# zhangxiaochen95/uav_bs_ctrl

Hardware: AMD Instinct MI355X
Metric: env-steps/sec (MADRQN, 8 UBS x 80 GT) (higher is better)
Workload: dtype f32

## Files before the change

include/uavgnn.h:

```cpp
#ifndef UAVGNN_H
#define UAVGNN_H

#include <stddef.h>
#include <stdint.h>

#ifdef __cplusplus
extern "C" {
#endif

#define UAVGNN_VERSION 101

#define UAVGNN_EINVAL (-1000)
#define UAVGNN_EUNSUPPORTED (-1001)
#define UAVGNN_EWORKSPACE (-1002)

typedef void* uavgnn_stream_t;

int uavgnn_version(void);

const char* uavgnn_strerror(int code);

int uavgnn_gatv2_fwd(const float* x_src, int E, int F_src, const float* x_dst, int F_dst, const int32_t* seg_off,
                     const int32_t* dst_order, int N, const float* W_s, const float* b_s, const float* W_d, const float* b_d, const float* attn,
                     const float* W_r, const float* b_r, int nh, int D, float slope, float* out, int ld_out,
// ... 117 lines not shown
int uavgnn_gemm_nt_h2(const float* X, int ldx, int K1, const float* X2, int ldx2, int M, int K, const float* rowmax, const float* rowmax2,
                      const void* planes, int N, const float* bias, float* Y, int ldy, int epilogue, uavgnn_stream_t stream);
int uavgnn_gemm_nt_h2_rm2(const float* X, int ldx, int K1, const float* X2, int ldx2, int M, int K, const float* rowmax, float* rowmax2_out,
                          const void* planes, int N, const float* bias, float* Y, int ldy, int epilogue, uavgnn_stream_t stream);
int uavgnn_gemm_nt_h2_n64(const float* X, int ldx, int M, int K, const float* rowmax, const void* planes, int N, float* Y, int ldy,
                          uavgnn_stream_t stream);
int uavgnn_gru_gates_bwd_fused_sums_rowmax(const float* pre, const float* h, const float* d_hout, const float* dq, int n_out,
                                           const float* W_out, int N, int H, float* d_gi, float* d_gh, float* d_h, float* col_sums,
                                           float* row_absmax, uavgnn_stream_t stream);
int uavgnn_relu_bwd_colsum_rowmax(const float* dy, long long ld, const float* y, long long ldy, float* out, long long ldo, int N, int C,
                                  float* acc, int S, float* row_absmax, uavgnn_stream_t stream);
int uavgnn_relu_bwd_colsum(const float* dy, long long ld, const float* y, long long ldy, float* out, long long ldo, int N, int C,
                           float* acc, int S, uavgnn_stream_t stream);

int uavgnn_flat_obs_supported(int H_out, int F);
int uavgnn_flat_obs_fwd(const float* agent, long long ld_a, int F_a, const float* gt, long long ld_g, int K_g, const float* ubs,
                        long long ld_u, int K_u, int rows, const float* W, const float* b, int H_out, float* y, long long ld_y,
                        uavgnn_stream_t stream);
int uavgnn_flat_obs_wgrad_chunks(long long rows, int H_out, int F);
int uavgnn_flat_obs_wgrad(const float* dy, long long ld_dy, int H_out, const float* agent, long long ld_a, int F_a, const float* gt,
                          long long ld_g, int K_g, const float* ubs, long long ld_u, int K_u, int rows, float* partials, int S,
                          int accumulate, uavgnn_stream_t stream);

int uavgnn_talk_attn_env_supported(int n_max, int M, int K);
int uavgnn_talk_attn_env_fwd(const float* s, int ld_s, const float* q, int ld_q, const float* v, int ld_v, int K, int M,
                             const int32_t* talk_off, const int32_t* talk_src, const int32_t* graph_off, int B,
                             int n_max, float scale, float* c, int ld_c, float* a_save, const float* x_copy, int ld_x,
                             int n_copy, uavgnn_stream_t stream);
int uavgnn_talk_attn_env_bwd(const float* s, int ld_s, const float* q, int ld_q, const float* v, int ld_v, int K, int M,
                             const int32_t* talk_off, const int32_t* talk_src, const int32_t* graph_off, int B,
                             int n_max, float scale, const float* a_save, const float* d_c, int ld_dc, float* d_s,
                             int ld_ds, float* d_q, int ld_dq, float* d_v, int ld_dv, uavgnn_stream_t stream);

int uavgnn_tarmac_msg_supported(int H, int M, int K, int n_ag);
long long uavgnn_tarmac_msg_weight_bytes(int H, int M, int K);
int uavgnn_tarmac_msg_prepare(const float* Wp, int ld, int H, int M, int K, void* tiles, uavgnn_stream_t stream);
int uavgnn_tarmac_msg_fwd(const float* x, int ld_x, const float* h, int ld_h, int N, int H, int n_ag, const void* tiles,
                          const float* bias, int M, int K, const int32_t* talk_off, const int32_t* talk_src, float scale,
                          float* c_out, int ld_c, float* a_save, float* proj_out, int ld_p, float* x_copy, int ld_xc,
                          uavgnn_stream_t stream);
int uavgnn_tarmac_msg_rowmax_supported(int H, int M, int K, int n_ag);
int uavgnn_tarmac_msg_fwd_rowmax(const float* x, int ld_x, const float* h, int ld_h, int N, int H, int n_ag, const void* tiles,
                                 const float* bias, int M, int K, const int32_t* talk_off, const int32_t* talk_src, float scale,
                                 float* c_out, int ld_c, float* a_save, float* proj_out, int ld_p, float* x_copy, int ld_xc,
                                 float* row_absmax, uavgnn_stream_t stream);

size_t uavgnn_degree_order_workspace_bytes(int N);
int uavgnn_degree_order(const int32_t* seg_off, int N, int32_t* order, void* workspace, size_t workspace_bytes,
                        uavgnn_stream_t stream);
size_t uavgnn_csc_transpose_workspace_bytes(int N);
int uavgnn_csc_transpose(const int32_t* talk_off, const int32_t* talk_src, int N, int E, int32_t* t_off,
                         int32_t* t_dst, int32_t* t_pos, void* workspace, size_t workspace_bytes,
                         uavgnn_stream_t stream);
int uavgnn_csc_transpose_env(const int32_t* talk_off, const int32_t* talk_src, const int32_t* graph_off, int B, int N,
                             int32_t* t_off, int32_t* t_dst, int32_t* t_pos, uavgnn_stream_t stream);

int uavgnn_adamw_polyak(float* p, float* g, float* exp_avg, float* exp_avg_sq, float* p_targ, long long n,
                        long long n_clip, const float* hyper, double beta1, double beta2, float eps, float weight_decay,
                        float clip, float polyak, uavgnn_stream_t stream);

int uavgnn_env_state_dim(int n_ubs, int n_gts, int fair_service);
int uavgnn_env_step(const int32_t* int_consts, const double* f64_consts, int B, const long long* actions,
                    const double* avail_moves, double* pos_ubs, const float* pos_gts, int32_t* prior, float* avg_rate,
                    int32_t* t, float* run_f32, double* n_colls, float* d_u2g, float* d_u2u, int32_t* gt_ubs,
                    int32_t* gt_rb, float* rate_per_gt, double* rate_per_ubs, int32_t* mask_collision, double* reward,
                    float* done, float* obs_gt, float* obs_ubs, float* obs_agent, float* state, uavgnn_stream_t stream);
// ... 105 lines not shown
```

uav_bs_ctrl_amd/csrc/f16x2.h:

```cpp
#pragma once
#include <hip/hip_runtime.h>

namespace uavgnn {
namespace h2 {

typedef float f32x2 __attribute__((ext_vector_type(2)));
typedef float f32x16 __attribute__((ext_vector_type(16)));
typedef _Float16 f16x2 __attribute__((ext_vector_type(2)));
typedef _Float16 f16x8 __attribute__((ext_vector_type(8)));
typedef unsigned u32x4 __attribute__((ext_vector_type(4)));
typedef unsigned u32x2 __attribute__((ext_vector_type(2)));

__device__ __forceinline__ int swz32(int row) { return (row >> 2) & 3; }
__device__ __forceinline__ f16x8 as_frag(u32x4 v) { return __builtin_bit_cast(f16x8, v); }
__device__ __forceinline__ f32x16 mfma32(f16x8 a, f16x8 b, f32x16 c) { return __builtin_amdgcn_mfma_f32_32x32x16_f16(a, b, c, 0, 0, 0); }

__device__ __forceinline__ int scale_exp(float amax) {
  const int e = static_cast<int>((__float_as_uint(amax) >> 23) & 0xffu);
  return max(-126, min(126, 14 - (e - 127)));
}
__device__ __forceinline__ float pow2f(int e) { return __uint_as_float(static_cast<unsigned>(e + 127) << 23); }

struct Split2 {
  unsigned hi, lo;
};
__device__ __forceinline__ Split2 split_pair(float x, float y) {
  Split2 s;
  const f16x2 h = __builtin_convertvector(f32x2{x, y}, f16x2);
  s.hi = __builtin_bit_cast(unsigned, h);
  const f32x2 r = f32x2{x, y} - __builtin_convertvector(h, f32x2);
  s.lo = __builtin_bit_cast(unsigned, __builtin_convertvector(r, f16x2));
  return s;
}
__device__ __forceinline__ void stage4(unsigned short* p, int plane_stride, float4 v, float s) {
  const Split2 a = split_pair(v.x * s, v.y * s), b = split_pair(v.z * s, v.w * s);
  *reinterpret_cast<u32x2*>(p) = u32x2{a.hi, b.hi};
  *reinterpret_cast<u32x2*>(p + plane_stride) = u32x2{a.lo, b.lo};
}
__device__ __forceinline__ void stage4(unsigned short* p, int plane_stride, float4 v, float4 s) {
  const Split2 a = split_pair(v.x * s.x, v.y * s.y), b = split_pair(v.z * s.z, v.w * s.w);
  *reinterpret_cast<u32x2*>(p) = u32x2{a.hi, b.hi};
  *reinterpret_cast<u32x2*>(p + plane_stride) = u32x2{a.lo, b.lo};
}

}
}
```

uav_bs_ctrl_amd/csrc/tarmac_msg.hip:

```cpp
#include <math.h>

#include "bf16x3.h"
#include "common.h"

namespace uavgnn {
namespace {

using namespace x3;

constexpr int kMsgWaves = 4;
constexpr int kMsgRows = 16 * kMsgWaves;
constexpr int kMsgThreads = kWave * kMsgWaves;
constexpr int kMaxCols = 128;

__device__ __forceinline__ bf16x8 frag_of(unsigned a, unsigned b, unsigned c, unsigned d) {
  return __builtin_bit_cast(bf16x8, u32x4{a, b, c, d});
}

__device__ __forceinline__ void lds_barrier() {
  __builtin_amdgcn_fence(__ATOMIC_RELEASE, "workgroup", "local");
  __builtin_amdgcn_s_barrier();
  __builtin_amdgcn_fence(__ATOMIC_ACQUIRE, "workgroup", "local");
}

struct Planes8 {
  u32x4 p[3];
};

__device__ __forceinline__ Planes8 split8(const float4 lo, const float4 hi) {
  const Split3 a = split_pair(lo.x, lo.y), b = split_pair(lo.z, lo.w), c = split_pair(hi.x, hi.y), d = split_pair(hi.z, hi.w);
  Planes8 r;
  r.p[0] = u32x4{a.h1, b.h1, c.h1, d.h1};
  r.p[1] = u32x4{a.h2, b.h2, c.h2, d.h2};
  r.p[2] = u32x4{a.h3, b.h3, c.h3, d.h3};
  return r;
}

__global__ __launch_bounds__(256) void tarmac_msg_prepare_kernel(const float* __restrict__ W, int ld, int R, int RP, int KK,
                                                                 u32x4* __restrict__ tiles) {
  const int idx = blockIdx.x * 256 + threadIdx.x;
  const int per_slice = RP * 4, nsl = KK / 32;
  if (idx >= nsl * per_slice) return;
  const int s = idx / per_slice, rem = idx - s * per_slice, r = rem >> 2, c = rem & 3;
  Planes8 pl;
  if (r < R) {
// ... 202 lines not shown
      }
      wave_sync_lds();
      msg_scatter(AD, NA, AV, SRC, DST, OFF, E, lane);
      wave_sync_lds();
      for (int c0 = 0; c0 < M; c0 += kWave) {
        const int ch = c0 + lane, chc = ch < M ? ch : M - 1;
        float v[NA];
#pragma unroll
        for (int t = 0; t < NA; ++t) v[t] = P[t * LDP + chc];
#pragma unroll 4
        for (int r = 0; r < NA; ++r) {
          float a = 0.f;
#pragma unroll
          for (int t = 0; t < NA; t += 4) {
            const float4 q = *reinterpret_cast<const float4*>(AD + r * NA + t);
            a = fmaf(q.x, v[t], a);
            a = fmaf(q.y, v[t + 1], a);
            a = fmaf(q.z, v[t + 2], a);
            a = fmaf(q.w, v[t + 3], a);
          }
          if (ch < M) P[r * LDP + ch] = a;
        }
      }
    }
  }
  wave_sync_lds();
  for (int r = 0; r < 16; ++r) {
    if (row0 + r >= N) break;
    float* d = c_out + static_cast<size_t>(row0 + r) * ld_c;
    for (int ch = lane; ch < M; ch += kWave) d[ch] = P[r * LDP + ch];
  }
}

template <int CT, bool TRAIN, bool RM = false>
__global__ __launch_bounds__(2 * kMsgThreads, 4) void tarmac_msg_fwd_k2_kernel(
    const float* __restrict__ x, int ld_x, const float* __restrict__ h, int ld_h, int N, int H, int n_ag,
    const u32x4* __restrict__ Wt, const float* __restrict__ bias, int M, int K, const int32_t* __restrict__ talk_off,
    const int32_t* __restrict__ talk_src, float scale, float* __restrict__ c_out, int ld_c, float* __restrict__ a_save,
    float* __restrict__ proj_out, int ld_p, float* __restrict__ x_copy, int ld_xc, float* __restrict__ row_absmax = nullptr) {
  constexpr int kThreads = 2 * kMsgThreads;
  __shared__ float sRowMax[kMsgWaves][2][16];
  float amax = 0.f;
  constexpr int RP = 16 * CT;
  constexpr int BCH = 3 * RP * 4;
  constexpr int BPT = (2 * BCH + kThreads - 1) / kThreads;
  constexpr int LDP = RP + 1;
  constexpr int NA = 16, EMAX = NA * NA;
  constexpr int kScratch = (NA + 4) + 5 * EMAX;
  constexpr int kLoopBytes = 2 * 2 * BCH * 16, kTailBytes = kMsgWaves * (16 * LDP + kScratch) * 4;
  __shared__ __attribute__((aligned(16))) unsigned char smem_raw[kLoopBytes > kTailBytes ? kLoopBytes : kTailBytes];
  u32x4(*sB)[2 * BCH] = reinterpret_cast<u32x4(*)[2 * BCH]>(smem_raw);

  const int tid = threadIdx.x, lane = tid & 63;
  const int wave = __builtin_amdgcn_readfirstlane(tid >> 6);
  const int tile = wave & 3, half = wave >> 2;
  const int j = lane & 15, g = lane >> 4;
  const int row0 = blockIdx.x * kMsgRows + tile * 16;
  const int row = row0 + j, rowc = min(row, N - 1);
  const int nsx = H / 32;
  const float* __restrict__ ar = (half ? h + static_cast<size_t>(rowc) * ld_h : x + static_cast<size_t>(rowc) * ld_x) + 4 * g;

  f32x4 acc[CT];
#pragma unroll
  for (int ct = 0; ct < CT; ++ct) acc[ct] = f32x4{0.f, 0.f, 0.f, 0.f};

  u32x4 rb[BPT];
  auto load_b = [&](int t) {
    t = min(t, nsx - 1);
// ... 66 lines not shown
    UAVGNN_MSG_STEP(a1_lo, a1_hi, t + 1)
  }
#undef UAVGNN_MSG_STEP
#undef UAVGNN_MSG_TERM
#undef UAVGNN_MSG_LOAD_A

  float* __restrict__ P = reinterpret_cast<float*>(smem_raw) + tile * (16 * LDP + kScratch);
  const int ncol = M + 2 * K;
  if (RM) load_fsrc();
  if (RM) {
    amax = fmaxf(amax, __shfl_xor(amax, 16));
    amax = fmaxf(amax, __shfl_xor(amax, 32));
    if (g == 0) sRowMax[tile][half][j] = amax;
  }
  if (half == 0) {
#pragma unroll
    for (int ct = 0; ct < CT; ++ct) {
      const int col = ct * 16 + j;
      const float b = col < ncol ? bias[col] : 0.f;
#pragma unroll
      for (int i = 0; i < 4; ++i) P[(4 * g + i) * LDP + col] = acc[ct][i] + b;
    }
  }
  lds_barrier();
  if (half == 1) {
#pragma unroll
    for (int ct = 0; ct < CT; ++ct) {
      const int col = ct * 16 + j;
#pragma unroll
      for (int i = 0; i < 4; ++i) P[(4 * g + i) * LDP + col] += acc[ct][i];
    }
  }
  lds_barrier();
  int* __restrict__ OFF = reinterpret_cast<int*>(P + 16 * LDP);
  float* __restrict__ SC = reinterpret_cast<float*>(OFF + NA + 4);
  float* __restrict__ AD = SC + EMAX;
  int* __restrict__ SRC = reinterpret_cast<int*>(AD + EMAX);
  int* __restrict__ DST = SRC + EMAX;
  float* __restrict__ AV = reinterpret_cast<float*>(DST + EMAX);
  if (half == 1) {
    if (TRAIN && proj_out != nullptr) {
      for (int r = 0; r < 16; ++r) {
        if (row0 + r >= N) break;
        float* d = proj_out + static_cast<size_t>(row0 + r) * ld_p;
        for (int col = lane; col < ncol; col += kWave) d[col] = P[r * LDP + col];
      }
    }
    lds_barrier();
    return;
  }
  bool poison = !ok;
  if (ok) {
    for (int i = lane; i < EMAX; i += kWave) AD[i] = 0.f;
    if (lane <= 16) OFF[lane] = toff - e_lo;
    wave_sync_lds();
    bool bad = false;
#pragma unroll
    for (int i = 0; i < 4; ++i) {
      const int e = lane + kWave * i;
      if (e < E) {
        const int u = fsrc[i] - row0;
        bad |= (u < 0) | (u >= 16);
        SRC[e] = u < 0 ? 0 : (u >= 16 ? 15 : u);
        int d = 0;
#pragma unroll
        for (int jj = 1; jj < 16; ++jj) d += e >= OFF[jj];
        DST[e] = d;
      }
    }
    poison = __any(bad);
    wave_sync_lds();
    if (!poison) {
      for (int e = lane; e < E; e += kWave) {
        const float* __restrict__ sr = P + SRC[e] * LDP + M;
        const float* __restrict__ qr = P + DST[e] * LDP + M + K;
        float a = 0.f;
#pragma unroll 4
        for (int k = 0; k < K; ++k) a = fmaf(sr[k], qr[k], a);
        SC[e] = a * scale;
      }
      wave_sync_lds();
      for (int e = lane; e < E; e += kWave) {
        const int d = DST[e];
        const int j0 = OFF[d], j1 = OFF[d + 1];
        float m = -INFINITY;
#pragma unroll 2
        for (int jj = j0; jj < j1; ++jj) m = fmaxf(m, SC[jj]);
        float den = 0.f;
#pragma unroll 2
        for (int jj = j0; jj < j1; ++jj) den += expf(SC[jj] - m);
        const float a = expf(SC[e] - m) / den;
        if (TRAIN && a_save != nullptr) a_save[e_lo + e] = a;
        AV[e] = a;
      }
      wave_sync_lds();
      msg_scatter(AD, NA, AV, SRC, DST, OFF, E, lane);
      wave_sync_lds();
    }
  }
  lds_barrier();
  if (poison) {
    for (int i = 0; i < 16; ++i)
      for (int ch = lane; ch < M; ch += kWave) P[i * LDP + ch] = NAN;
  } else {
    for (int c0 = 0; c0 < M; c0 += kWave) {
      const int ch = c0 + lane, chc = ch < M ? ch : M - 1;
      float v[NA];
#pragma unroll
      for (int t = 0; t < NA; ++t) v[t] = P[t * LDP + chc];
#pragma unroll 4
      for (int r = 0; r < NA; ++r) {
        float a = 0.f;
#pragma unroll
        for (int t = 0; t < NA; t += 4) {
          const float4 q = *reinterpret_cast<const float4*>(AD + r * NA + t);
          a = fmaf(q.x, v[t], a);
          a = fmaf(q.y, v[t + 1], a);
          a = fmaf(q.z, v[t + 2], a);
          a = fmaf(q.w, v[t + 3], a);
        }
        if (ch < M) P[r * LDP + ch] = a;
      }
    }
  }
  wave_sync_lds();
  for (int r = 0; r < 16; ++r) {
    if (row0 + r >= N) break;
    float* d = c_out + static_cast<size_t>(row0 + r) * ld_c;
    for (int ch = lane; ch < M; ch += kWave) d[ch] = P[r * LDP + ch];
  }
  if (RM) {
    float cm = 0.f;
    for (int ch = g; ch < M; ch += 4) cm = fmaxf(cm, fabsf(P[j * LDP + ch]));
    cm = fmaxf(cm, __shfl_xor(cm, 16));
    cm = fmaxf(cm, __shfl_xor(cm, 32));
    if (g == 0 && row < N) row_absmax[row] = fmaxf(cm, fmaxf(sRowMax[tile][0][j], sRowMax[tile][1][j]));
  }
}

}
}

using namespace uavgnn;

extern "C" int uavgnn_tarmac_msg_supported(int H, int M, int K, int n_ag) {
  if (H < 32 || (H % 32) || M < 1 || K < 1 || K > 64 || M + 2 * K > kMaxCols) return 0;
  if (n_ag < 1 || n_ag > 16 || (16 % n_ag)) return 0;
  return 1;
}

static int msg_rows_padded(int M, int K) {
  const int ct = (M + 2 * K + 15) / 16;
  return 16 * (ct <= 4 ? 4 : ct <= 6 ? 6 : 8);
}

extern "C" long long uavgnn_tarmac_msg_weight_bytes(int H, int M, int K) {
  if (H <= 0 || M <= 0 || K <= 0 || M + 2 * K > kMaxCols) return 0;
  return static_cast<long long>(2 * H / 32) * 3 * msg_rows_padded(M, K) * 64;
}

extern "C" int uavgnn_tarmac_msg_prepare(const float* Wp, int ld, int H, int M, int K, void* tiles, uavgnn_stream_t stream) {
  if (!Wp || !tiles || H <= 0 || M <= 0 || K <= 0 || ld < 2 * H) return UAVGNN_EINVAL;
  if ((H % 32) || (ld & 3) || (reinterpret_cast<uintptr_t>(Wp) & 15) || (reinterpret_cast<uintptr_t>(tiles) & 15) || M + 2 * K > kMaxCols)
    return UAVGNN_EUNSUPPORTED;
  const int R = M + 2 * K, RP = msg_rows_padded(M, K), KK = 2 * H;
  const int total = (KK / 32) * RP * 4;
  hipLaunchKernelGGL(tarmac_msg_prepare_kernel, dim3((total + 255) / 256), dim3(256), 0, static_cast<hipStream_t>(stream), Wp, ld,
                     R, RP, KK, static_cast<u32x4*>(tiles));
  return launch_status();
}

static int msg_launch(const float* x, int ld_x, const float* h, int ld_h, int N, int H, int n_ag, const void* tiles, const float* bias, int M,
                      int K, const int32_t* talk_off, const int32_t* talk_src, float scale, float* c_out, int ld_c, float* a_save,
                      float* proj_out, int ld_p, float* x_copy, int ld_xc, float* row_absmax, uavgnn_stream_t stream) {
  if (N < 0 || !x || !h || !tiles || !bias || !talk_off || !c_out || ld_x < H || ld_h < H || ld_c < M) return UAVGNN_EINVAL;
  if (proj_out && ld_p < M + 2 * K) return UAVGNN_EINVAL;
  if (x_copy && ld_xc < H) return UAVGNN_EINVAL;
  if (!uavgnn_tarmac_msg_supported(H, M, K, n_ag) || (N % n_ag) || (ld_x & 3) || (ld_h & 3) || (x_copy && (ld_xc & 3)) ||
      ((reinterpret_cast<uintptr_t>(x) | reinterpret_cast<uintptr_t>(h) | reinterpret_cast<uintptr_t>(tiles) |
        reinterpret_cast<uintptr_t>(x_copy)) & 15))
    return UAVGNN_EUNSUPPORTED;
  if (N == 0) return 0;
  const int ct = (M + 2 * K + 15) / 16;
  const bool train = a_save != nullptr || proj_out != nullptr || x_copy != nullptr;
  const dim3 grid((N + kMsgRows - 1) / kMsgRows), block(kMsgThreads);
  hipStream_t st = static_cast<hipStream_t>(stream);
  const u32x4* Wt = static_cast<const u32x4*>(tiles);
  if (row_absmax != nullptr && ct > 6) return UAVGNN_EUNSUPPORTED;
  if (ct <= 6) {
    const dim3 block2(2 * kMsgThreads);
#define UAVGNN_MSG_K2(CT_, TR_)                                                                                                        \
  {                                                                                                                                    \
    if (row_absmax != nullptr)                                                                                                         \
      hipLaunchKernelGGL((tarmac_msg_fwd_k2_kernel<CT_, TR_, true>), grid, block2, 0, st, x, ld_x, h, ld_h, N, H, n_ag, Wt, bias, M, K, \
                         talk_off, talk_src, scale, c_out, ld_c, a_save, proj_out, ld_p, x_copy, ld_xc, row_absmax);                   \
    else                                                                                                                               \
      hipLaunchKernelGGL((tarmac_msg_fwd_k2_kernel<CT_, TR_, false>), grid, block2, 0, st, x, ld_x, h, ld_h, N, H, n_ag, Wt, bias, M, K, \
                         talk_off, talk_src, scale, c_out, ld_c, a_save, proj_out, ld_p, x_copy, ld_xc, nullptr);                      \
  }
    if (ct <= 4) {
      if (train) UAVGNN_MSG_K2(4, true)
      else UAVGNN_MSG_K2(4, false)
    } else {
      if (train) UAVGNN_MSG_K2(6, true)
      else UAVGNN_MSG_K2(6, false)
    }
#undef UAVGNN_MSG_K2
    return launch_status();
  }
#define UAVGNN_MSG_K1(TR_)                                                                                                   \
  hipLaunchKernelGGL((tarmac_msg_fwd_kernel<TR_>), grid, block, 0, st, x, ld_x, h, ld_h, N, H, n_ag, Wt, bias, M, K, talk_off, \
                     talk_src, scale, c_out, ld_c, a_save, proj_out, ld_p, x_copy, ld_xc)
  if (train) UAVGNN_MSG_K1(true);
  else UAVGNN_MSG_K1(false);
#undef UAVGNN_MSG_K1
  return launch_status();
}

extern "C" int uavgnn_tarmac_msg_rowmax_supported(int H, int M, int K, int n_ag) {
  return (uavgnn_tarmac_msg_supported(H, M, K, n_ag) && (M + 2 * K + 15) / 16 <= 6) ? 1 : 0;
}

extern "C" int uavgnn_tarmac_msg_fwd_rowmax(const float* x, int ld_x, const float* h, int ld_h, int N, int H, int n_ag, const void* tiles,
                                            const float* bias, int M, int K, const int32_t* talk_off, const int32_t* talk_src,
                                            float scale, float* c_out, int ld_c, float* a_save, float* proj_out, int ld_p,
                                            float* x_copy, int ld_xc, float* row_absmax, uavgnn_stream_t stream) {
  if (!row_absmax) return UAVGNN_EINVAL;
  return msg_launch(x, ld_x, h, ld_h, N, H, n_ag, tiles, bias, M, K, talk_off, talk_src, scale, c_out, ld_c, a_save, proj_out, ld_p, x_copy,
                    ld_xc, row_absmax, stream);
}

extern "C" int uavgnn_tarmac_msg_fwd(const float* x, int ld_x, const float* h, int ld_h, int N, int H, int n_ag, const void* tiles,
                                     const float* bias, int M, int K, const int32_t* talk_off, const int32_t* talk_src,
                                     float scale, float* c_out, int ld_c, float* a_save, float* proj_out, int ld_p,
                                     float* x_copy, int ld_xc, uavgnn_stream_t stream) {
  return msg_launch(x, ld_x, h, ld_h, N, H, n_ag, tiles, bias, M, K, talk_off, talk_src, scale, c_out, ld_c, a_save, proj_out, ld_p, x_copy,
                    ld_xc, nullptr, stream);
}
```

uav_bs_ctrl_amd/ops.py:

```python
from __future__ import annotations

import os
import torch as th

from . import _lib as L

NEG_SLOPE = 0.2
K1_IMAGE = os.environ.get("UAVGNN_K1_IMAGE", "1") != "0"
HETERO_FUSED = True
K1_BF16Z = os.environ.get("UAVGNN_K1_BF16Z", "1") != "0"
K1_ROWMAX = os.environ.get("UAVGNN_K1_ROWMAX", "1") != "0"
K1_ROWMAX_MIN_ROWS = 1 << 17
K1_ROWMAX_DENSE_DEG = int(os.environ.get("UAVGNN_K1_ROWMAX_DENSE_DEG", "16"))
K1_ROWMAX_DENSE_MIN_ROWS = 16384


class _KernelTimer:

    def __init__(self):
        self.enabled = False
        self.only = None
        self._spans = {}

    def reset(self, enabled=True, only=None):
# ... 1169 lines not shown
    p.grad[start:start + g.shape[0]].add_(g)


class _TimeSplit(th.autograd.Function):

    @staticmethod
    def forward(ctx, x_all, T1, holder):
        N = x_all.shape[0] // T1
        buf = th.empty((T1, N, x_all.shape[1]), dtype=x_all.dtype, device=x_all.device)
        holder.append(buf)
        ctx.buf = buf
        return tuple(x_all.detach().view(T1, N, -1).unbind(0))

    @staticmethod
    def backward(ctx, *grads):
        buf = ctx.buf
        for t, g in enumerate(grads):
            if g is None:
                buf[t].zero_()
            elif g.data_ptr() != buf[t].data_ptr() or g.stride() != buf[t].stride():
                buf[t].copy_(g)
        return buf.view(-1, buf.shape[2]), None, None


def time_split(x_all, T1):
    if not (th.is_grad_enabled() and x_all.requires_grad):
        return x_all.view(T1, x_all.shape[0] // T1, -1).unbind(0), [None] * T1
    holder = []
    xs = _TimeSplit.apply(x_all, T1, holder)
    return xs, list(holder[0].unbind(0))


MSG_FUSED = os.environ.get("UAVGNN_MSG_FUSED", "1") != "0"


def _tarmac_msg_plan(x, h, Wp, bp, M, K, env, N, H):
    if not MSG_FUSED or env is None or N == 0:
        return None
    _, B, n_ag = env
    if N != B * n_ag or (H + M) % 4 or not L.lib().uavgnn_tarmac_msg_supported(H, M, K, n_ag):
        return None
    if (Wp.shape != (M + 2 * K, 2 * H) or not Wp.is_contiguous() or Wp.data_ptr() % 16 or not bp.is_contiguous()
            or x.data_ptr() % 16 or h.data_ptr() % 16 or x.dtype != th.float32 or Wp.dtype != th.float32):
        return None
    lib = L.lib()
    tiles = _weight_planes("msgw", (Wp,), (H, M, K), lib.uavgnn_tarmac_msg_weight_bytes(H, M, K),
                           lambda buf: L.check(lib.uavgnn_tarmac_msg_prepare(Wp.data_ptr(), Wp.stride(0), H, M, K, buf.data_ptr(),
                                                                            L.stream()), "uavgnn_tarmac_msg_prepare"))
    return tiles, n_ag


def _launch_tarmac_msg(msg, x, h, bp, M, K, talk_off, talk_src, N, H, c_ptr, ld_c, a_save, proj, ld_p, x_copy, ld_xc, rowmax=None):
    tiles, n_ag = msg
    entry, outs = ("uavgnn_tarmac_msg_fwd", ()) if rowmax is None else ("uavgnn_tarmac_msg_fwd_rowmax", (rowmax.data_ptr(),))
    with KERNEL_TIMER.span("tarmac_msg_fwd", (N, H, M, K, int(proj is not None), int(x_copy is not None))):
        rc = getattr(L.lib(), entry)(x.data_ptr(), x.stride(0), h.data_ptr(), h.stride(0), N, H, n_ag, tiles.data_ptr(), bp.data_ptr(), M, K,
                                     L.ptr(talk_off), L.ptr(talk_src), 1.0 / K, c_ptr, ld_c, a_save, proj, ld_p, x_copy, ld_xc, *outs,
                                     L.stream())
    L.check(rc, entry)


DUEL_FUSED = True


def dueling_params(layer):
    return layer.adv_head.weight, layer.adv_head.bias, layer.v_head.weight, layer.v_head.bias


def dueling_fold(W_adv, b_adv, w_v, b_v):
    return W_adv - W_adv.mean(0, keepdim=True) + w_v, b_adv - b_adv.mean() + b_v


def dueling_split(G, g):
    dWa, dwv = (None, None) if G is None else (G - G.mean(0, keepdim=True), G.sum(0, keepdim=True))
    dba, dbv = (None, None) if g is None else (g - g.mean(), g.sum().reshape(1))
    return dWa, dba, dwv, dbv


def dueling_supported(h, W_adv, b_adv, w_v, b_v) -> bool:
    return bool(DUEL_FUSED and h.is_cuda and h.dtype == th.float32 and h.dim() == 2 and h.shape[0] > 0 and _mc_operand(h)
                and all(t.is_cuda and t.dtype == th.float32 and t.is_contiguous() for t in (W_adv, b_adv, w_v, b_v))
                and W_adv.data_ptr() % 16 == 0 and w_v.data_ptr() % 16 == 0
                and L.lib().uavgnn_head_duel_supported(h.shape[1], W_adv.shape[0]))


def _duel_weff(W_adv, w_v):
    A, H = W_adv.shape
    Wa, wv = W_adv.detach(), w_v.detach()

# ... 393 lines not shown
```

Measured before the change: 2.682 million.

## Use scaled fp16x2 split MFMA path for TarMAC message projection

Measured after the change: 2.708 million, median of 6. No clear change (+1.0%).

```diff
diff --git a/include/uavgnn.h b/include/uavgnn.h
--- a/include/uavgnn.h
+++ b/include/uavgnn.h
@@ -173,6 +173,7 @@
                              int n_max, float scale, const float* a_save, const float* d_c, int ld_dc, float* d_s,
                              int ld_ds, float* d_q, int ld_dq, float* d_v, int ld_dv, uavgnn_stream_t stream);
 
+#define UAVGNN_MSG_BF16X3 (1 << 30)
 int uavgnn_tarmac_msg_supported(int H, int M, int K, int n_ag);
 long long uavgnn_tarmac_msg_weight_bytes(int H, int M, int K);
 int uavgnn_tarmac_msg_prepare(const float* Wp, int ld, int H, int M, int K, void* tiles, uavgnn_stream_t stream);
diff --git a/uav_bs_ctrl_amd/csrc/f16x2.h b/uav_bs_ctrl_amd/csrc/f16x2.h
--- a/uav_bs_ctrl_amd/csrc/f16x2.h
+++ b/uav_bs_ctrl_amd/csrc/f16x2.h
@@ -32,6 +32,24 @@
   s.lo = __builtin_bit_cast(unsigned, __builtin_convertvector(r, f16x2));
   return s;
 }
+typedef float f32x4 __attribute__((ext_vector_type(4)));
+__device__ __forceinline__ f32x4 mfma16(f16x8 a, f16x8 b, f32x4 c) { return __builtin_amdgcn_mfma_f32_16x16x32_f16(a, b, c, 0, 0, 0); }
+
+__device__ __forceinline__ unsigned abs_bits(float v) { return __float_as_uint(v) & 0x7fffffffu; }
+__device__ __forceinline__ unsigned max_abs_bits(unsigned m, float4 v) {
+  return max(max(m, max(abs_bits(v.x), abs_bits(v.y))), max(abs_bits(v.z), abs_bits(v.w)));
+}
+__device__ __forceinline__ float bound_of_bits(unsigned m) { return m > 0x7f800000u ? __uint_as_float(0x7f800000u) : __uint_as_float(m); }
+
+struct Frag2 {
+  u32x4 hi, lo;
+};
+__device__ __forceinline__ Frag2 split8(float4 a, float4 b, float s) {
+  const Split2 p0 = split_pair(a.x * s, a.y * s), p1 = split_pair(a.z * s, a.w * s);
+  const Split2 p2 = split_pair(b.x * s, b.y * s), p3 = split_pair(b.z * s, b.w * s);
+  return Frag2{u32x4{p0.hi, p1.hi, p2.hi, p3.hi}, u32x4{p0.lo, p1.lo, p2.lo, p3.lo}};
+}
+
 __device__ __forceinline__ void stage4(unsigned short* p, int plane_stride, float4 v, float s) {
   const Split2 a = split_pair(v.x * s, v.y * s), b = split_pair(v.z * s, v.w * s);
   *reinterpret_cast<u32x2*>(p) = u32x2{a.hi, b.hi};
diff --git a/uav_bs_ctrl_amd/csrc/tarmac_msg.hip b/uav_bs_ctrl_amd/csrc/tarmac_msg.hip
--- a/uav_bs_ctrl_amd/csrc/tarmac_msg.hip
+++ b/uav_bs_ctrl_amd/csrc/tarmac_msg.hip
@@ -2,6 +2,7 @@
 
 #include "bf16x3.h"
 #include "common.h"
+#include "f16x2.h"
 
 namespace uavgnn {
 namespace {
@@ -11,6 +12,7 @@
 constexpr int kMsgWaves = 4;
 constexpr int kMsgRows = 16 * kMsgWaves;
 constexpr int kMsgThreads = kWave * kMsgWaves;
+constexpr int kMsgResident = 2;
 constexpr int kMaxCols = 128;
 
 __device__ __forceinline__ bf16x8 frag_of(unsigned a, unsigned b, unsigned c, unsigned d) {
@@ -279,8 +281,122 @@
   }
 }
 
+template <int CT, bool TRAIN, bool RM>
+__device__ __forceinline__ void msg_pair_tail(float* __restrict__ P, int half, int lane, int row0, int N, int M, int K, int toff, int e_lo,
+                                              int E, bool ok, const int (&fsrc)[4], float scale, float* __restrict__ c_out, int ld_c,
+                                              float* __restrict__ a_save, float* __restrict__ proj_out, int ld_p,
+                                              float* __restrict__ row_absmax, const float (*rowmax_xh)[16]) {
+  constexpr int LDP = 16 * CT + 1;
+  constexpr int NA = 16, EMAX = NA * NA;
+  const int ncol = M + 2 * K, j = lane & 15, g = lane >> 4, row = row0 + j;
+  int* __restrict__ OFF = reinterpret_cast<int*>(P + 16 * LDP);
+  float* __restrict__ SC = reinterpret_cast<float*>(OFF + NA + 4);
+  float* __restrict__ AD = SC + EMAX;
+  int* __restrict__ SRC = reinterpret_cast<int*>(AD + EMAX);
+  int* __restrict__ DST = SRC + EMAX;
+  float* __restrict__ AV = reinterpret_cast<float*>(DST + EMAX);
+  if (half == 1) {
+    if (TRAIN && proj_out != nullptr) {
+      for (int r = 0; r < 16; ++r) {
+        if (row0 + r >= N) break;
+        float* d = proj_out + static_cast<size_t>(row0 + r) * ld_p;
+        for (int col = lane; col < ncol; col += kWave) d[col] = P[r * LDP + col];
+      }
+    }
+    lds_barrier();
+    return;
+  }
+  bool poison = !ok;
+  if (ok) {
+    for (int i = lane; i < EMAX; i += kWave) AD[i] = 0.f;
+    if (lane <= 16) OFF[lane] = toff - e_lo;
+    wave_sync_lds();
+    bool bad = false;
+#pragma unroll
+    for (int i = 0; i < 4; ++i) {
+      const int e = lane + kWave * i;
+      if (e < E) {
+        const int u = fsrc[i] - row0;
+        bad |= (u < 0) | (u >= 16);
+        SRC[e] = u < 0 ? 0 : (u >= 16 ? 15 : u);
+        int d = 0;
+#pragma unroll
+        for (int jj = 1; jj < 16; ++jj) d += e >= OFF[jj];
+        DST[e] = d;
+      }
+    }
+    poison = __any(bad);
+    wave_sync_lds();
+    if (!poison) {
+      for (int e = lane; e < E; e += kWave) {
+        const float* __restrict__ sr = P + SRC[e] * LDP + M;
+        const float* __restrict__ qr = P + DST[e] * LDP + M + K;
+        float a = 0.f;
+#pragma unroll 4
+        for (int k = 0; k < K; ++k) a = fmaf(sr[k], qr[k], a);
+        SC[e] = a * scale;
+      }
+      wave_sync_lds();
+      for (int e = lane; e < E; e += kWave) {
+        const int d = DST[e];
+        const int j0 = OFF[d], j1 = OFF[d + 1];
+        float m = -INFINITY;
+#pragma unroll 2
+        for (int jj = j0; jj < j1; ++jj) m = fmaxf(m, SC[jj]);
+        float den = 0.f;
+#pragma unroll 2
+        for (int jj = j0; jj < j1; ++jj) den += expf(SC[jj] - m);
+        const float a = expf(SC[e] - m) / den;
+        if (TRAIN && a_save != nullptr) a_save[e_lo + e] = a;
+        AV[e] = a;
+      }
+      wave_sync_lds();
+      msg_scatter(AD, NA, AV, SRC, DST, OFF, E, lane);
+      wave_sync_lds();
+    }
+  }
+  lds_barrier();
+  if (poison) {
+    for (int i = 0; i < 16; ++i)
+      for (int ch = lane; ch < M; ch += kWave) P[i * LDP + ch] = NAN;
+  } else {
+    for (int c0 = 0; c0 < M; c0 += kWave) {
+      const int ch = c0 + lane, chc = ch < M ? ch : M - 1;
+      float v[NA];
+#pragma unroll
+      for (int t = 0; t < NA; ++t) v[t] = P[t * LDP + chc];
+#pragma unroll 4
+      for (int r = 0; r < NA; ++r) {
+        float a = 0.f;
+#pragma unroll
+        for (int t = 0; t < NA; t += 4) {
+          const float4 q = *reinterpret_cast<const float4*>(AD + r * NA + t);
+          a = fmaf(q.x, v[t], a);
+          a = fmaf(q.y, v[t + 1], a);
+          a = fmaf(q.z, v[t + 2], a);
+          a = fmaf(q.w, v[t + 3], a);
+        }
+        if (ch < M) P[r * LDP + ch] = a;
+      }
+    }
+  }
+  wave_sync_lds();
+  for (int r = 0; r < 16; ++r) {
+    if (row0 + r >= N) break;
+    float* d = c_out + static_cast<size_t>(row0 + r) * ld_c;
+    for (int ch = lane; ch < M; ch += kWave) d[ch] = P[r * LDP + ch];
+  }
+  if (RM) {
+    float cm = 0.f;
+    for (int ch = g; ch < M; ch += 4) cm = fmaxf(cm, fabsf(P[j * LDP + ch]));
+    cm = fmaxf(cm, __shfl_xor(cm, 16));
+    cm = fmaxf(cm, __shfl_xor(cm, 32));
+    if (g == 0 && row < N) row_absmax[row] = fmaxf(cm, fmaxf(rowmax_xh[0][j], rowmax_xh[1][j]));
+  }
+}
+
 template <int CT, bool TRAIN, bool RM = false>
-__global__ __launch_bounds__(2 * kMsgThreads, 4) void tarmac_msg_fwd_k2_kernel(
+__global__ __launch_bounds__(2 * kMsgThreads, 4) void tarmac_msg_fwd_k2_x3_kernel(
     const float* __restrict__ x, int ld_x, const float* __restrict__ h, int ld_h, int N, int H, int n_ag,
     const u32x4* __restrict__ Wt, const float* __restrict__ bias, int M, int K, const int32_t* __restrict__ talk_off,
     const int32_t* __restrict__ talk_src, float scale, float* __restrict__ c_out, int ld_c, float* __restrict__ a_save,
@@ -413,110 +529,187 @@
     }
   }
   lds_barrier();
-  int* __restrict__ OFF = reinterpret_cast<int*>(P + 16 * LDP);
-  float* __restrict__ SC = reinterpret_cast<float*>(OFF + NA + 4);
-  float* __restrict__ AD = SC + EMAX;
-  int* __restrict__ SRC = reinterpret_cast<int*>(AD + EMAX);
-  int* __restrict__ DST = SRC + EMAX;
-  float* __restrict__ AV = reinterpret_cast<float*>(DST + EMAX);
+  msg_pair_tail<CT, TRAIN, RM>(P, half, lane, row0, N, M, K, toff, e_lo, E, ok, fsrc, scale, c_out, ld_c, a_save, proj_out, ld_p, row_absmax,
+                               sRowMax[tile]);
+}
+
+template <int CT, bool TRAIN, bool RM, int RES>
+__global__ __launch_bounds__(2 * kMsgThreads, 4) void tarmac_msg_fwd_k2_kernel(
+    const float* __restrict__ x, int ld_x, const float* __restrict__ h, int ld_h, int N, int H, int n_ag,
+    const u32x4* __restrict__ Wt, const float* __restrict__ bias, int M, int K, const int32_t* __restrict__ talk_off,
+    const int32_t* __restrict__ talk_src, float scale, float* __restrict__ c_out, int ld_c, float* __restrict__ a_save,
+    float* __restrict__ proj_out, int ld_p, float* __restrict__ x_copy, int ld_xc, float* __restrict__ row_absmax) {
+  constexpr int kThreads = 2 * kMsgThreads;
+  __shared__ float sRowMax[kMsgWaves][2][16];
+  constexpr int RP = 16 * CT;
+  constexpr int BCH = 2 * RP * 4;
+  constexpr int BPT = (2 * BCH + kThreads - 1) / kThreads;
+  constexpr int LDP = RP + 1;
+  constexpr int NA = 16, EMAX = NA * NA;
+  constexpr int kScratch = (NA + 4) + 5 * EMAX;
+  constexpr int kLoopBytes = 2 * 2 * BCH * 16, kTailBytes = kMsgWaves * (16 * LDP + kScratch) * 4;
+  __shared__ __attribute__((aligned(16))) unsigned char smem_raw[kLoopBytes > kTailBytes ? kLoopBytes : kTailBytes];
+  u32x4(*sB)[2 * BCH] = reinterpret_cast<u32x4(*)[2 * BCH]>(smem_raw);
+
+  const int tid = threadIdx.x, lane = tid & 63;
+  const int wave = __builtin_amdgcn_readfirstlane(tid >> 6);
+  const int tile = wave & 3, half = wave >> 2;
+  const int j = lane & 15, g = lane >> 4;
+  const int row0 = blockIdx.x * kMsgRows + tile * 16;
+  const int row = row0 + j, rowc = min(row, N - 1);
+  const int nsx = H / 32;
+  const float* __restrict__ ar = (half ? h + static_cast<size_t>(rowc) * ld_h : x + static_cast<size_t>(rowc) * ld_x) + 4 * g;
+  const float* __restrict__ cinv = reinterpret_cast<const float*>(Wt + static_cast<size_t>(2 * nsx) * BCH);
+
+  f32x4 acc[CT];
+#pragma unroll
+  for (int ct = 0; ct < CT; ++ct) acc[ct] = f32x4{0.f, 0.f, 0.f, 0.f};
+
+  u32x4 rb[BPT];
+  auto load_b = [&](int t) {
+    t = min(t, nsx - 1);
+#pragma unroll
+    for (int i = 0; i < BPT; ++i) {
+      const int q = min(tid + kThreads * i, 2 * BCH - 1);
+      rb[i] = Wt[static_cast<size_t>(q < BCH ? t : nsx + t) * BCH + (q < BCH ? q : q - BCH)];
+    }
+  };
+  auto store_b = [&](int buf) {
+#pragma unroll
+    for (int i = 0; i < BPT; ++i) sB[buf][min(tid + kThreads * i, 2 * BCH - 1)] = rb[i];
+  };
+  auto load_a = [&](float4& lo, float4& hi, int s) {
+    const float* p_ = ar + 32 * s;
+    lo = *reinterpret_cast<const float4*>(p_);
+    hi = *reinterpret_cast<const float4*>(p_ + 16);
+  };
+
+  const int toff = half == 0 ? talk_off[min(row0 + min(lane, 16), N)] : 0;
+  load_b(0);
+  __builtin_amdgcn_sched_barrier(0);
+  float4 a_lo[RES], a_hi[RES];
+#pragma unroll
+  for (int r = 0; r < RES; ++r) load_a(a_lo[r], a_hi[r], min(r, nsx - 1));
+  __builtin_amdgcn_sched_barrier(0);
+  const int e_lo = __shfl(toff, 0);
+  const int E = __shfl(toff, 16) - e_lo;
+  const bool ok = E <= EMAX && E >= 0;
+  store_b(0);
+  load_b(1);
+  lds_barrier();
+
+#define UAVGNN_MSG_TERM(FA, PB)                                                                                                   \
+  acc[cp] = h2::mfma16(FA, h2::as_frag(sb[(PB) * RP * 4 + (cp * 16 + j) * 4 + (g ^ swz(j))]), acc[cp]);                           \
+  acc[cp + 1] = h2::mfma16(FA, h2::as_frag(sb[(PB) * RP * 4 + ((cp + 1) * 16 + j) * 4 + (g ^ swz(j))]), acc[cp + 1]);
+  unsigned mb = 0u;
+  int se = 0;
+  for (int t0 = 0; t0 < nsx; t0 += RES) {
+    unsigned gm = mb;
+#pragma unroll
+    for (int r = 0; r < RES; ++r) gm = h2::max_abs_bits(h2::max_abs_bits(gm, a_lo[r]), a_hi[r]);
+    gm = max(gm, static_cast<unsigned>(__shfl_xor(static_cast<int>(gm), 16)));
+    gm = max(gm, static_cast<unsigned>(__shfl_xor(static_cast<int>(gm), 32)));
+    const int se_new = h2::scale_exp(__uint_as_float(gm));
+    if (t0 > 0) {
+      const float f = h2::pow2f(max(se_new - se, -127));
+#pragma unroll
+      for (int i = 0; i < 4; ++i) {
+        const float fi = __shfl(f, 4 * g + i);
+#pragma unroll
+        for (int ct = 0; ct < CT; ++ct) acc[ct][i] *= fi;
+      }
+    }
+    mb = gm;
+    se = se_new;
+    const float sc = h2::pow2f(se);
+    h2::Frag2 pa[RES];
+#pragma unroll
+    for (int r = 0; r < RES; ++r) {
+      const int t = t0 + r;
+      pa[r] = h2::split8(a_lo[r], a_hi[r], sc);
+      if (TRAIN && half == 0 && x_copy != nullptr && row < N && t < nsx) {
+        float* d = x_copy + static_cast<size_t>(row) * ld_xc + 32 * t + 4 * g;
+        *reinterpret_cast<float4*>(d) = a_lo[r];
+        *reinterpret_cast<float4*>(d + 16) = a_hi[r];
+      }
+      if (t + RES < nsx) load_a(a_lo[r], a_hi[r], t + RES);
+    }
+#pragma unroll
+    for (int r = 0; r < RES; ++r) {
+      const int t = t0 + r;
+      if (t < nsx) {
+        const h2::f16x8 fh = h2::as_frag(pa[r].hi), fl = h2::as_frag(pa[r].lo);
+        const u32x4* sb = sB[t & 1] + half * BCH;
+#pragma unroll
+        for (int cp = 0; cp < CT; cp += 2) {
+          UAVGNN_MSG_TERM(fh, 1) UAVGNN_MSG_TERM(fl, 0) UAVGNN_MSG_TERM(fh, 0)
+        }
+        store_b((t + 1) & 1);
+        load_b(t + 2);
+        lds_barrier();
+      }
+    }
+  }
+#undef UAVGNN_MSG_TERM
+  if (RM && g == 0) sRowMax[tile][half][j] = h2::bound_of_bits(mb);
+
+  float* __restrict__ P = reinterpret_cast<float*>(smem_raw) + tile * (16 * LDP + kScratch);
+  const int ncol = M + 2 * K;
+  int fsrc[4];
+#pragma unroll
+  for (int i = 0; i < 4; ++i) fsrc[i] = (half == 0 && ok && lane + kWave * i < E) ? talk_src[e_lo + lane + kWave * i] : 0;
+  const float rinv = h2::pow2f(-se);
+  float ri[4];
+#pragma unroll
+  for (int i = 0; i < 4; ++i) ri[i] = __shfl(rinv, 4 * g + i);
+  if (half == 0) {
+#pragma unroll
+    for (int ct = 0; ct < CT; ++ct) {
+      const int col = ct * 16 + j;
+      const float b = col < ncol ? bias[col] : 0.f, ci = cinv[col];
+#pragma unroll
+      for (int i = 0; i < 4; ++i) P[(4 * g + i) * LDP + col] = acc[ct][i] * ri[i] * ci + b;
+    }
+  }
+  lds_barrier();
   if (half == 1) {
-    if (TRAIN && proj_out != nullptr) {
-      for (int r = 0; r < 16; ++r) {
-        if (row0 + r >= N) break;
-        float* d = proj_out + static_cast<size_t>(row0 + r) * ld_p;
-        for (int col = lane; col < ncol; col += kWave) d[col] = P[r * LDP + col];
-      }
-    }
-    lds_barrier();
-    return;
-  }
-  bool poison = !ok;
-  if (ok) {
-    for (int i = lane; i < EMAX; i += kWave) AD[i] = 0.f;
-    if (lane <= 16) OFF[lane] = toff - e_lo;
-    wave_sync_lds();
-    bool bad = false;
-#pragma unroll
-    for (int i = 0; i < 4; ++i) {
-      const int e = lane + kWave * i;
-      if (e < E) {
-        const int u = fsrc[i] - row0;
-        bad |= (u < 0) | (u >= 16);
-        SRC[e] = u < 0 ? 0 : (u >= 16 ? 15 : u);
-        int d = 0;
-#pragma unroll
-        for (int jj = 1; jj < 16; ++jj) d += e >= OFF[jj];
-        DST[e] = d;
-      }
-    }
-    poison = __any(bad);
-    wave_sync_lds();
-    if (!poison) {
-      for (int e = lane; e < E; e += kWave) {
-        const float* __restrict__ sr = P + SRC[e] * LDP + M;
-        const float* __restrict__ qr = P + DST[e] * LDP + M + K;
-        float a = 0.f;
-#pragma unroll 4
-        for (int k = 0; k < K; ++k) a = fmaf(sr[k], qr[k], a);
-        SC[e] = a * scale;
-      }
-      wave_sync_lds();
-      for (int e = lane; e < E; e += kWave) {
-        const int d = DST[e];
-        const int j0 = OFF[d], j1 = OFF[d + 1];
-        float m = -INFINITY;
-#pragma unroll 2
-        for (int jj = j0; jj < j1; ++jj) m = fmaxf(m, SC[jj]);
-        float den = 0.f;
-#pragma unroll 2
-        for (int jj = j0; jj < j1; ++jj) den += expf(SC[jj] - m);
-        const float a = expf(SC[e] - m) / den;
-        if (TRAIN && a_save != nullptr) a_save[e_lo + e] = a;
-        AV[e] = a;
-      }
-      wave_sync_lds();
-      msg_scatter(AD, NA, AV, SRC, DST, OFF, E, lane);
-      wave_sync_lds();
+#pragma unroll
+    for (int ct = 0; ct < CT; ++ct) {
+      const int col = ct * 16 + j;
+      const float ci = cinv[col];
+#pragma unroll
+      for (int i = 0; i < 4; ++i) P[(4 * g + i) * LDP + col] += acc[ct][i] * ri[i] * ci;
     }
   }
   lds_barrier();
-  if (poison) {
-    for (int i = 0; i < 16; ++i)
-      for (int ch = lane; ch < M; ch += kWave) P[i * LDP + ch] = NAN;
-  } else {
-    for (int c0 = 0; c0 < M; c0 += kWave) {
-      const int ch = c0 + lane, chc = ch < M ? ch : M - 1;
-      float v[NA];
-#pragma unroll
-      for (int t = 0; t < NA; ++t) v[t] = P[t * LDP + chc];
-#pragma unroll 4
-      for (int r = 0; r < NA; ++r) {
-        float a = 0.f;
-#pragma unroll
-        for (int t = 0; t < NA; t += 4) {
-          const float4 q = *reinterpret_cast<const float4*>(AD + r * NA + t);
-          a = fmaf(q.x, v[t], a);
-          a = fmaf(q.y, v[t + 1], a);
-          a = fmaf(q.z, v[t + 2], a);
-          a = fmaf(q.w, v[t + 3], a);
-        }
-        if (ch < M) P[r * LDP + ch] = a;
-      }
-    }
-  }
-  wave_sync_lds();
-  for (int r = 0; r < 16; ++r) {
-    if (row0 + r >= N) break;
-    float* d = c_out + static_cast<size_t>(row0 + r) * ld_c;
-    for (int ch = lane; ch < M; ch += kWave) d[ch] = P[r * LDP + ch];
-  }
-  if (RM) {
-    float cm = 0.f;
-    for (int ch = g; ch < M; ch += 4) cm = fmaxf(cm, fabsf(P[j * LDP + ch]));
-    cm = fmaxf(cm, __shfl_xor(cm, 16));
-    cm = fmaxf(cm, __shfl_xor(cm, 32));
-    if (g == 0 && row < N) row_absmax[row] = fmaxf(cm, fmaxf(sRowMax[tile][0][j], sRowMax[tile][1][j]));
-  }
+  msg_pair_tail<CT, TRAIN, RM>(P, half, lane, row0, N, M, K, toff, e_lo, E, ok, fsrc, scale, c_out, ld_c, a_save, proj_out, ld_p, row_absmax,
+                               sRowMax[tile]);
+}
+
+__global__ __launch_bounds__(256) void tarmac_msg_prepare_h2_kernel(const float* __restrict__ W, int ld, int R, int RP, int KK,
+                                                                    u32x4* __restrict__ tiles) {
+  __shared__ float red[4];
+  const int r = blockIdx.x, tid = threadIdx.x;
+  const int per_plane = RP * 4, nsl = KK / 32;
+  const float* wr = W + static_cast<size_t>(min(r, R - 1)) * ld;
+  float m = 0.f;
+  for (int i = tid; i < KK; i += 256) m = fmaxf(m, fabsf(wr[i]));
+  m = wave_max(m);
+  if ((tid & 63) == 0) red[tid >> 6] = m;
+  __syncthreads();
+  m = fmaxf(fmaxf(red[0], red[1]), fmaxf(red[2], red[3]));
+  const int se = h2::scale_exp(m);
+  const float s = r < R ? h2::pow2f(se) : 0.f;
+  for (int q = tid; q < nsl * 4; q += 256) {
+    const int sl = q >> 2, c = q & 3;
+    const float* src = wr + 32 * sl + 4 * c;
+    h2::Frag2 f = h2::split8(*reinterpret_cast<const float4*>(src), *reinterpret_cast<const float4*>(src + 16), s);
+    if (r >= R) f.hi = f.lo = u32x4{0u, 0u, 0u, 0u};
+    u32x4* dst = tiles + static_cast<size_t>(sl) * 2 * per_plane + r * 4 + (c ^ swz(r));
+    dst[0] = f.hi;
+    dst[per_plane] = f.lo;
+  }
+  if (tid == 0) reinterpret_cast<float*>(tiles + static_cast<size_t>(nsl) * 2 * per_plane)[r] = r < R ? h2::pow2f(-se) : 1.f;
 }
 
 }
@@ -525,6 +718,7 @@
 using namespace uavgnn;
 
 extern "C" int uavgnn_tarmac_msg_supported(int H, int M, int K, int n_ag) {
+  K &= ~UAVGNN_MSG_BF16X3;
   if (H < 32 || (H % 32) || M < 1 || K < 1 || K > 64 || M + 2 * K > kMaxCols) return 0;
   if (n_ag < 1 || n_ag > 16 || (16 % n_ag)) return 0;
   return 1;
@@ -535,16 +729,28 @@
   return 16 * (ct <= 4 ? 4 : ct <= 6 ? 6 : 8);
 }
 
+static bool msg_h2(int M, int K, bool bf16x3) { return !bf16x3 && (M + 2 * K + 15) / 16 <= 6; }
+
 extern "C" long long uavgnn_tarmac_msg_weight_bytes(int H, int M, int K) {
+  const bool x3 = (K & UAVGNN_MSG_BF16X3) != 0;
+  K &= ~UAVGNN_MSG_BF16X3;
   if (H <= 0 || M <= 0 || K <= 0 || M + 2 * K > kMaxCols) return 0;
-  return static_cast<long long>(2 * H / 32) * 3 * msg_rows_padded(M, K) * 64;
+  const long long rp = msg_rows_padded(M, K);
+  return msg_h2(M, K, x3) ? static_cast<long long>(2 * H / 32) * 2 * rp * 64 + rp * 4 : static_cast<long long>(2 * H / 32) * 3 * rp * 64;
 }
 
 extern "C" int uavgnn_tarmac_msg_prepare(const float* Wp, int ld, int H, int M, int K, void* tiles, uavgnn_stream_t stream) {
+  const bool x3 = (K & UAVGNN_MSG_BF16X3) != 0;
+  K &= ~UAVGNN_MSG_BF16X3;
   if (!Wp || !tiles || H <= 0 || M <= 0 || K <= 0 || ld < 2 * H) return UAVGNN_EINVAL;
   if ((H % 32) || (ld & 3) || (reinterpret_cast<uintptr_t>(Wp) & 15) || (reinterpret_cast<uintptr_t>(tiles) & 15) || M + 2 * K > kMaxCols)
     return UAVGNN_EUNSUPPORTED;
   const int R = M + 2 * K, RP = msg_rows_padded(M, K), KK = 2 * H;
+  if (msg_h2(M, K, x3)) {
+    hipLaunchKernelGGL(tarmac_msg_prepare_h2_kernel, dim3(RP), dim3(256), 0, static_cast<hipStream_t>(stream), Wp, ld, R, RP, KK,
+                       static_cast<u32x4*>(tiles));
+    return launch_status();
+  }
   const int total = (KK / 32) * RP * 4;
   hipLaunchKernelGGL(tarmac_msg_prepare_kernel, dim3((total + 255) / 256), dim3(256), 0, static_cast<hipStream_t>(stream), Wp, ld,
                      R, RP, KK, static_cast<u32x4*>(tiles));
@@ -552,8 +758,10 @@
 }
 
 static int msg_launch(const float* x, int ld_x, const float* h, int ld_h, int N, int H, int n_ag, const void* tiles, const float* bias, int M,
-                      int K, const int32_t* talk_off, const int32_t* talk_src, float scale, float* c_out, int ld_c, float* a_save,
+                      int K_fmt, const int32_t* talk_off, const int32_t* talk_src, float scale, float* c_out, int ld_c, float* a_save,
                       float* proj_out, int ld_p, float* x_copy, int ld_xc, float* row_absmax, uavgnn_stream_t stream) {
+  const bool x3 = (K_fmt & UAVGNN_MSG_BF16X3) != 0;
+  const int K = K_fmt & ~UAVGNN_MSG_BF16X3;
   if (N < 0 || !x || !h || !tiles || !bias || !talk_off || !c_out || ld_x < H || ld_h < H || ld_c < M) return UAVGNN_EINVAL;
   if (proj_out && ld_p < M + 2 * K) return UAVGNN_EINVAL;
   if (x_copy && ld_xc < H) return UAVGNN_EINVAL;
@@ -570,14 +778,18 @@
   if (row_absmax != nullptr && ct > 6) return UAVGNN_EUNSUPPORTED;
   if (ct <= 6) {
     const dim3 block2(2 * kMsgThreads);
-#define UAVGNN_MSG_K2(CT_, TR_)                                                                                                        \
-  {                                                                                                                                    \
-    if (row_absmax != nullptr)                                                                                                         \
-      hipLaunchKernelGGL((tarmac_msg_fwd_k2_kernel<CT_, TR_, true>), grid, block2, 0, st, x, ld_x, h, ld_h, N, H, n_ag, Wt, bias, M, K, \
-                         talk_off, talk_src, scale, c_out, ld_c, a_save, proj_out, ld_p, x_copy, ld_xc, row_absmax);                   \
-    else                                                                                                                               \
-      hipLaunchKernelGGL((tarmac_msg_fwd_k2_kernel<CT_, TR_, false>), grid, block2, 0, st, x, ld_x, h, ld_h, N, H, n_ag, Wt, bias, M, K, \
-                         talk_off, talk_src, scale, c_out, ld_c, a_save, proj_out, ld_p, x_copy, ld_xc, nullptr);                      \
+#define UAVGNN_MSG_K2_(...)                                                                                                           \
+  hipLaunchKernelGGL((__VA_ARGS__), grid, block2, 0, st, x, ld_x, h, ld_h, N, H, n_ag, Wt, bias, M, K, talk_off, talk_src, scale, c_out, ld_c, \
+                     a_save, proj_out, ld_p, x_copy, ld_xc, row_absmax)
+#define UAVGNN_MSG_K2(CT_, TR_)                                                                           \
+  {                                                                                                       \
+    if (x3) {                                                                                             \
+      if (row_absmax != nullptr) UAVGNN_MSG_K2_(tarmac_msg_fwd_k2_x3_kernel<CT_, TR_, true>);             \
+      else UAVGNN_MSG_K2_(tarmac_msg_fwd_k2_x3_kernel<CT_, TR_, false>);                                  \
+    } else {                                                                                              \
+      if (row_absmax != nullptr) UAVGNN_MSG_K2_(tarmac_msg_fwd_k2_kernel<CT_, TR_, true, kMsgResident>);  \
+      else UAVGNN_MSG_K2_(tarmac_msg_fwd_k2_kernel<CT_, TR_, false, kMsgResident>);                       \
+    }                                                                                                     \
   }
     if (ct <= 4) {
       if (train) UAVGNN_MSG_K2(4, true)
@@ -587,6 +799,7 @@
       else UAVGNN_MSG_K2(6, false)
     }
 #undef UAVGNN_MSG_K2
+#undef UAVGNN_MSG_K2_
     return launch_status();
   }
 #define UAVGNN_MSG_K1(TR_)                                                                                                   \
@@ -599,6 +812,7 @@
 }
 
 extern "C" int uavgnn_tarmac_msg_rowmax_supported(int H, int M, int K, int n_ag) {
+  K &= ~UAVGNN_MSG_BF16X3;
   return (uavgnn_tarmac_msg_supported(H, M, K, n_ag) && (M + 2 * K + 15) / 16 <= 6) ? 1 : 0;
 }
 
diff --git a/uav_bs_ctrl_amd/ops.py b/uav_bs_ctrl_amd/ops.py
--- a/uav_bs_ctrl_amd/ops.py
+++ b/uav_bs_ctrl_amd/ops.py
@@ -1225,6 +1225,8 @@
 
 
 MSG_FUSED = os.environ.get("UAVGNN_MSG_FUSED", "1") != "0"
+MSG_H2 = True
+_MSG_BF16X3 = 1 << 30
 
 
 def _tarmac_msg_plan(x, h, Wp, bp, M, K, env, N, H):
@@ -1237,17 +1239,18 @@
             or x.data_ptr() % 16 or h.data_ptr() % 16 or x.dtype != th.float32 or Wp.dtype != th.float32):
         return None
     lib = L.lib()
-    tiles = _weight_planes("msgw", (Wp,), (H, M, K), lib.uavgnn_tarmac_msg_weight_bytes(H, M, K),
-                           lambda buf: L.check(lib.uavgnn_tarmac_msg_prepare(Wp.data_ptr(), Wp.stride(0), H, M, K, buf.data_ptr(),
+    Kf = K if MSG_H2 else K | _MSG_BF16X3
+    tiles = _weight_planes("msgw", (Wp,), (H, M, Kf), lib.uavgnn_tarmac_msg_weight_bytes(H, M, Kf),
+                           lambda buf: L.check(lib.uavgnn_tarmac_msg_prepare(Wp.data_ptr(), Wp.stride(0), H, M, Kf, buf.data_ptr(),
                                                                             L.stream()), "uavgnn_tarmac_msg_prepare"))
-    return tiles, n_ag
+    return tiles, n_ag, Kf
 
 
 def _launch_tarmac_msg(msg, x, h, bp, M, K, talk_off, talk_src, N, H, c_ptr, ld_c, a_save, proj, ld_p, x_copy, ld_xc, rowmax=None):
-    tiles, n_ag = msg
+    tiles, n_ag, Kf = msg
     entry, outs = ("uavgnn_tarmac_msg_fwd", ()) if rowmax is None else ("uavgnn_tarmac_msg_fwd_rowmax", (rowmax.data_ptr(),))
     with KERNEL_TIMER.span("tarmac_msg_fwd", (N, H, M, K, int(proj is not None), int(x_copy is not None))):
-        rc = getattr(L.lib(), entry)(x.data_ptr(), x.stride(0), h.data_ptr(), h.stride(0), N, H, n_ag, tiles.data_ptr(), bp.data_ptr(), M, K,
+        rc = getattr(L.lib(), entry)(x.data_ptr(), x.stride(0), h.data_ptr(), h.stride(0), N, H, n_ag, tiles.data_ptr(), bp.data_ptr(), M, Kf,
                                      L.ptr(talk_off), L.ptr(talk_src), 1.0 / K, c_ptr, ld_c, a_save, proj, ld_p, x_copy, ld_xc, *outs,
                                      L.stream())
     L.check(rc, entry)
```
